# boyuanf/tensorflow_train_distributed

Measured on AMD Instinct MI355X. Metric: images/sec (whole node) ResNet-50 bf16 MirroredStrategy at 1/2/4/8 MI355X, higher is better.
Workload: dtype bf16; 1 GPU; model=ResNet-50 v1.5, global_batch=1024, per_gpu_batch=1024, image_size=224, parallelism=dp1, optimizer=momentum-SGD 0.9, wd 5e-5, fp32 master, precision=bf16, hipgraph=True

## Files before the change

tensorflow_train_distributed_amd/csrc/kernels/conv_dgrad.hip:

```cpp
#include "gemm_conv.h"

TTDK_EXPORT int ttdk_conv_dgrad(const bf16_t* dy, const bf16_t* wt, const TtdkConv* g, int bm, int bn,
                                const TtdkEpilogue* epi, hipStream_t st) {
  if (g->K % 8) return hipErrorInvalidValue;
  EpiParams pe = to_epi(epi);
  if (pe.by && (pe.stat == nullptr || pe.mode != 0 || g->C % 8 || pe.ldo % 8 || pe.residual || pe.act))
    return hipErrorInvalidValue;
  if ((pe.by2 || pe.stat2) && !(pe.by && pe.by2 && pe.stat2)) return hipErrorInvalidValue;
  const int N = g->C, K = g->R * g->S * g->K;
  DenseParams pb{wt, K, N, K};
  if (g->R == 1 && g->S == 1 && g->ph == 0 && g->pw == 0) {
    const int M = g->N * g->P * g->Q;
    DenseParams pa{dy, g->K, M, K};
    if (g->sh != 1 || g->sw != 1) {
      if (g->sh != g->sw || pe.bH) return hipErrorInvalidValue;
      pe.remap = 1;
      pe.rP = g->P;
      pe.rQ = g->Q;
      pe.rOH = g->H;
      pe.rOW = g->W;
      pe.rs = g->sh;
    }
    const int bbn = big_bn(M, N, K);
    if (((bm == 0 && pe.stat == nullptr) || bm == 256) && bbn && (bm != 256 || bn == bbn))
      return bbn == 256 ? big::dense<256>(dy, g->K, true, wt, K, true, pe, M, N, K, 1, st)
                        : big::dense<128>(dy, g->K, true, wt, K, true, pe, M, N, K, 1, st);
    if (bm == 256 && pe.stat) return hipErrorInvalidValue;
    if (bm == 0 || bn == 0 || bm == 256) pick_tile(M, N, &bm, &bn);
    return dispatch<KDense, KDense>(&pa, &pb, pe, M, N, K, 1, bm, bn, st);
  }
  const int M = g->N * g->H * g->W;
  const int bbn = big_bn(M, N, K);
  static const bool strided_big = [] {
    const char* e = getenv("TTD_BIG_STRIDED_DGRAD");
    return e != nullptr && e[0] == '1';
  }();
  const bool unit = g->sh == 1 && g->sw == 1;
  if (((bm == 0 && pe.stat == nullptr) || bm == 256) && bbn && (bm != 256 || bn == bbn) && g->K % 64 == 0 &&
      !pe.remap && (unit || strided_big)) {
    const big::ConvP pa = conv_params(dy, g->P, g->Q, g->K, g->H, g->W, g, M);
    const big::DenseP pb2{wt, K, N};
    if (unit) {
      if (bbn == 256)
        return big::launch<256, big::OpConvK<128, 2, true, true>, big::OpDenseK<128, 2>>(pa, pb2, pe, M, N, K, 1, st);
      return big::launch<128, big::OpConvK<128, 2, true, true>, big::OpDenseK<64, 2>>(pa, pb2, pe, M, N, K, 1, st);
    }
    if (bbn == 256)
      return big::launch<256, big::OpConvK<128, 2, true>, big::OpDenseK<128, 2>>(pa, pb2, pe, M, N, K, 1, st);
    return big::launch<128, big::OpConvK<128, 2, true>, big::OpDenseK<64, 2>>(pa, pb2, pe, M, N, K, 1, st);
  }
  if (bm == 256 && pe.stat) return hipErrorInvalidValue;
  if (bm == 0 || bn == 0 || bm == 256) pick_tile(M, N, &bm, &bn);
  GatherParams pa{dy, g->P, g->Q, g->K, g->H, g->W, g->R, g->S, g->sh, g->sw, g->ph, g->pw, g->dh, g->dw, M, K};
  return dispatch<KConvDgrad, KDense>(&pa, &pb, pe, M, N, K, 1, bm, bn, st);
}

TTDK_EXPORT int ttdk_conv_dgrad_bnpro(const bf16_t* g_in, const bf16_t* wt, const TtdkConv* g, const bf16_t* y,
                                      const float* coef, bf16_t* dz, const TtdkEpilogue* epi, hipStream_t st) {
  if (!plan::conv_dgrad_bnpro_takes(*g)) return hipErrorNotSupported;
  EpiParams pe = to_epi(epi);
  if (pe.by && (pe.stat == nullptr || pe.mode != 0 || g->C % 8 || pe.ldo % 8 || pe.residual || pe.act))
    return hipErrorInvalidValue;
  if ((pe.by2 || pe.stat2) && !(pe.by && pe.by2 && pe.stat2)) return hipErrorInvalidValue;
  const int N = g->C, K = g->K;
  const int M = g->N * g->P * g->Q;
  const int bbn = big_bn(M, N, K);
  if (pe.mode != 0 || pe.remap) return hipErrorNotSupported;
  pe.py = y;
  pe.pcoef = coef;
  pe.pdz = dz;
  pe.pld = K;
  const big::DenseP pa{g_in, K, M}, pb{wt, K, N};
  if (bbn == 256)
    return big::launch<256, big::OpDenseKBN<128, 2>, big::OpDenseK<128, 2>, 0, 0>(pa, pb, pe, M, N, K, 1, st);
  return big::launch<128, big::OpDenseKBN<128, 2>, big::OpDenseK<64, 2>, 0, 0>(pa, pb, pe, M, N, K, 1, st);
}

__global__ __launch_bounds__(256) void subpixel_weights_kernel(const bf16_t* __restrict__ wt, bf16_t* __restrict__ ws,
                                                               int C, int R, int S, int Kc, int s, int r0, int Tr,
                                                               int s0, int Ts) {
  const int k8n = Kc >> 3;
  const long long total = static_cast<long long>(C) * Tr * Ts * k8n;
  for (long long idx = blockIdx.x * 256LL + threadIdx.x; idx < total; idx += static_cast<long long>(gridDim.x) * 256) {
    const int k8 = static_cast<int>(idx % k8n);
    long long rest = idx / k8n;
    const int ts = static_cast<int>(rest % Ts);
    rest /= Ts;
    const int tr = static_cast<int>(rest % Tr);
    const long long c = rest / Tr;
    const bf16_t* src = wt + c * (static_cast<long long>(R) * S * Kc) +
                        (static_cast<long long>(r0 + tr * s) * S + (s0 + ts * s)) * Kc + k8 * 8;
    reinterpret_cast<uint4*>(ws)[idx] = *reinterpret_cast<const uint4*>(src);
  }
}

TTDK_EXPORT int ttdk_conv_dgrad_subpixel(const bf16_t* dy, const bf16_t* wt, const TtdkConv* g, bf16_t* ws,
                                         int ws_ready, const TtdkEpilogue* epi, hipStream_t st) {
  const int s = g->sh;
  if (g->sw != s || s < 2 || g->dh != 1 || g->dw != 1 || g->R < s || g->S < s || g->K % 8 || g->C % 8)
    return hipErrorInvalidValue;
  EpiParams pe = to_epi(epi);
  if (pe.remap || pe.residual || pe.aux || pe.mode == 1 || pe.by2 || pe.stat2 || pe.bH) return hipErrorInvalidValue;
  if ((pe.stat != nullptr) != (pe.by != nullptr) || (pe.by && (pe.mode != 0 || g->C % 8 || pe.ldo % 8)))
    return hipErrorInvalidValue;
  const int N = g->C, Kc = g->K;
  const size_t esz = pe.mode == 0 ? sizeof(bf16_t) : sizeof(float);
// ... 47 lines not shown
```

tensorflow_train_distributed_amd/csrc/kernels/gemm_conv.h:

```cpp
#pragma once
#include "common.h"
#include "gemm_plan.h"

#include <algorithm>
#include <cstdlib>
#include <type_traits>

namespace ttdk_rt {
int& pers_flag();
int& reserved_cus();
int& fold_flag();
}

namespace ttdk {
namespace {

using plan::big_bn;
using plan::big_bn_wgrad;
using plan::pick_tile;

constexpr int BK = 64;
constexpr int NTHR = 256;

__device__ __forceinline__ int kmaj_off(int row, int chunk) { return row * 128 + ((chunk ^ ((row >> 1) & 7)) << 4); }
// ... 1819 lines not shown
        if (E.stat2) r8[j] += __shfl_xor(r8[j], o, 64);
      }
    }
    float* red = reinterpret_cast<float*>(smem + BM * PITCH);
    if (lane < CPR) {
#pragma unroll
      for (int j = 0; j < 8; ++j) {
        red[(wave * 3 + 0) * BN + c * 8 + j] = s8[j];
        red[(wave * 3 + 1) * BN + c * 8 + j] = q8[j];
        red[(wave * 3 + 2) * BN + c * 8 + j] = r8[j];
      }
    }
    __syncthreads();
    for (int t2 = tid; t2 < BN; t2 += T) {
      if (n0 + t2 < N) {
        float ss = 0.f, qq = 0.f, rr = 0.f;
#pragma unroll
        for (int k = 0; k < NW; ++k) {
          ss += red[(k * 3 + 0) * BN + t2];
          qq += red[(k * 3 + 1) * BN + t2];
          rr += red[(k * 3 + 2) * BN + t2];
        }
        E.stat[(static_cast<long long>(tile_m) * 2 + 0) * N + n0 + t2] = ss;
        E.stat[(static_cast<long long>(tile_m) * 2 + 1) * N + n0 + t2] = qq;
        if (E.stat2) {
          E.stat2[(static_cast<long long>(tile_m) * 2 + 0) * N + n0 + t2] = ss;
          E.stat2[(static_cast<long long>(tile_m) * 2 + 1) * N + n0 + t2] = rr;
        }
      }
    }
  }
}


constexpr int kEkBias = 1, kEkDGelu = 2, kEkBeta = 4, kEkAux = 8, kEkGelu = 16;

template <int EK, bool CHECK, int BNH, int WC>
__device__ __forceinline__ void pers_epi(const f32x4_t (&acc)[2][2][4][2], const EpiParams& E, int m0, int n0, int M,
                                         int N, float alpha, int lane, int wm, int wn) {
  const int g = lane >> 4, i16 = lane & 15;
  const bool odd = g & 1;
  bf16_t* const out = static_cast<bf16_t*>(E.out);
  constexpr bool LD = (EK & (kEkDGelu | kEkBeta)) != 0;
  uint2 rvb[2][2][2], ovb[2][2][2];
  auto load_blk = [&](int it, uint2 (&rv)[2][2], uint2 (&ov)[2][2]) {
    const int ha = it >> 2, a = it & 3;
    const int m = m0 + ha * 128 + wm * 64 + a * 16 + i16;
    if (CHECK && m >= M) return;
#pragma unroll
    for (int hb = 0; hb < 2; ++hb) {
      const int nb = n0 + hb * BNH + wn * WC + 4 * g;
#pragma unroll
      for (int b = 0; b < 2; ++b) {
        if constexpr ((EK & kEkDGelu) != 0)
          if (!CHECK || nb + 16 * b < N)
            rv[hb][b] = *reinterpret_cast<const uint2*>(E.residual + static_cast<long long>(m) * E.ldr + nb + 16 * b);
        if constexpr ((EK & kEkBeta) != 0)
          if (!CHECK || nb + 16 * b < N)
            ov[hb][b] = *reinterpret_cast<const uint2*>(out + static_cast<long long>(m) * E.ldo + nb + 16 * b);
      }
    }
  };
  if constexpr (LD) load_blk(0, rvb[0], ovb[0]);
#pragma unroll
  for (int it = 0; it < 8; ++it) {
    const int ha = it >> 2, a = it & 3;
// ... 208 lines not shown
    if (atomicAdd(tq + 8, 1) == static_cast<int>(gridDim.x) - 1) {
#pragma unroll
      for (int i = 0; i < 9; ++i) tq[i] = 0;
    }
  }
}

constexpr int kMaxCtr = 1 << 16;
inline int* tile_counters(hipStream_t st, int tiles) {
  if (tiles > kMaxCtr - 16) return nullptr;
  struct Buf {
    hipStream_t st;
    int* p;
  };
  static Buf bufs[16] = {};
  for (auto& b : bufs)
    if (b.p && b.st == st) return b.p;
  for (auto& b : bufs) {
    if (!b.p) {
      if (hipMalloc(&b.p, kMaxCtr * sizeof(int)) != hipSuccess) return b.p = nullptr, nullptr;
      if (hipMemsetAsync(b.p, 0, kMaxCtr * sizeof(int), st) != hipSuccess) return nullptr;
      b.st = st;
      return b.p;
    }
  }
  return nullptr;
}

inline bool inkernel_fold() { return ::ttdk_rt::fold_flag() != 0; }

inline int device_cus_total() {
  static int cus = [] {
    int dev = 0, n = 0;
    hipGetDevice(&dev);
    if (hipDeviceGetAttribute(&n, hipDeviceAttributeMultiprocessorCount, dev) != hipSuccess || n <= 0) n = 256;
    return n;
  }();
  return cus;
}

inline int device_cus() {
  const int total = device_cus_total();
  const int r = ::ttdk_rt::reserved_cus();
  return (r > 0 && total - r >= total / 2) ? total - r : total;
}

template <int BN, class OA, class OB, int F8 = 0, int PP = 0>
hipError_t launch(const typename OA::Params& pa, const typename OB::Params& pb, const EpiParams& pe, int M, int N,
                  int K, int splits, hipStream_t st) {
  const int tm = ceil_div(M, BM), tn = ceil_div(N, BN);
  const int ktiles = K / (F8 ? 128 : 64);
  const int cus = device_cus();
  const int tiles = tm * tn;
  splits = plan::clamp_splits(ktiles, splits);
  const int per = ceil_div(ktiles, splits);
  if constexpr (F8 == 0 && PP == 1 && OA::THREADS == THR && BN == 256) {
    int ek = -1;
    if (pe.act == kActNone && !pe.residual) ek = 0;
    else if (pe.act == kActGelu && !pe.residual) ek = kEkGelu;
    else if (pe.act == kActDGelu && pe.residual) ek = kEkDGelu;
    if (ek >= 0) {
      if (pe.bias) ek |= kEkBias;
      if (pe.beta) ek |= kEkBeta;
      if (pe.aux) ek |= kEkAux;
    }
    if (::ttdk_rt::pers_flag() && splits == 1 && pe.mode == 0 && !pe.remap && !pe.stat && !pe.by && !pe.bH && tiles > cus &&
        N % 8 == 0 && pe.ldo % 8 == 0 && (!pe.residual || pe.ldr % 4 == 0) && (!pe.bias || al16(pe.bias)) &&
        al16(pe.out) && (!pe.aux || al16(pe.aux)) && (!pe.residual || (reinterpret_cast<uintptr_t>(pe.residual) & 7) == 0)) {
      const int ovl = ::ttdk_rt::pers_flag() == 1;
      static const int fullwait = getenv_int("TTD_PERS_STORE_WAIT", 0);
      static const int queue = getenv_int("TTD_PERS_QUEUE", 1);
      int* tq = nullptr;
      if (queue && cus % 8 == 0) {
        int* c = tile_counters(st, 0);
        if (c) tq = c + kMaxCtr - 16;
      }
#define TTDK_PERS(EKV)                                                                                                \
  case EKV:                                                                                                           \
    hipLaunchKernelGGL((gemm256p_kernel<BN, OA, OB, EKV>), dim3(cus), dim3(THR), 0, st, pa, pb, pe, M, N, K, tm, tn, ovl, \
                       fullwait, tq);                                                                                 \
    return hipGetLastError();
      switch (ek) {
        TTDK_PERS(0)
        TTDK_PERS(kEkBias)
        TTDK_PERS(kEkBias | kEkAux | kEkGelu)
        TTDK_PERS(kEkDGelu)
        TTDK_PERS(kEkBeta)
        default: break;
      }
#undef TTDK_PERS
    }
  }
  hipLaunchKernelGGL((gemm256_kernel<BN, OA, OB, F8, PP>), dim3(tm * tn, splits), dim3(OA::THREADS), 0, st, pa, pb, pe, M, N,
                     K, tm, tn, per, 0);
  return hipGetLastError();
}

template <int BN, int PP>
hipError_t dense_pp(const bf16_t* A, long long lda, bool ak, const bf16_t* B, long long ldb, bool bk,
                    const EpiParams& pe, int M, int N, int K, int splits, hipStream_t st) {
  DenseP pa{A, lda, M}, pb{B, ldb, N};
  constexpr int BH = BN / 2;
  if (ak && bk) return launch<BN, OpDenseK<128, 2>, OpDenseK<BH, 2>, 0, PP>(pa, pb, pe, M, N, K, splits, st);
  if (ak) return launch<BN, OpDenseKU<128, 2>, OpDenseMN<BH>, 0, PP>(pa, pb, pe, M, N, K, splits, st);
  if (bk) return launch<BN, OpDenseMN<128>, OpDenseKU<BH, 2>, 0, PP>(pa, pb, pe, M, N, K, splits, st);
  return launch<BN, OpDenseMN<128>, OpDenseMN<BH>, 0, PP>(pa, pb, pe, M, N, K, splits, st);
}

inline hipError_t dense_rowsum(const bf16_t* A, long long lda, const bf16_t* B, long long ldb, const EpiParams& pe,
                               int M, int N, int K, int splits, hipStream_t st) {
  DenseP pa{A, lda, M}, pb{B, ldb, N};
  const int tm = ceil_div(M, BM), tn = ceil_div(N, 256);
  const int ktiles = K / 64;
  splits = plan::clamp_splits(ktiles, splits);
  const int per = ceil_div(ktiles, splits);
  hipLaunchKernelGGL((gemm256_kernel<256, OpDenseMN<128>, OpDenseMN<128>, 0, 1, 1>), dim3(tm * tn, splits), dim3(THR), 0,
                     st, pa, pb, pe, M, N, K, tm, tn, per, 0);
  return hipGetLastError();
}

template <int BN>
hipError_t dense(const bf16_t* A, long long lda, bool ak, const bf16_t* B, long long ldb, bool bk,
                 const EpiParams& pe, int M, int N, int K, int splits, hipStream_t st) {
  if constexpr (BN == 256) {
    static const int pp_on = getenv_int("TTD_BIG_PP", 1);
    const int kts = K / 64 / (splits > 1 ? splits : 1);
    if (kts >= 16 && pp_on)
// ... 131 lines not shown
```

tensorflow_train_distributed_amd/csrc/kernels/gemm_plan.h:

```cpp
#pragma once

struct TtdkConv {
  int N, H, W, C;
  int K, R, S;
  int P, Q;
  int sh, sw, ph, pw, dh, dw;
};

namespace ttdk {
namespace plan {

inline int cdiv(long long a, long long b) { return static_cast<int>((a + b - 1) / b); }

inline bool is_pointwise(const TtdkConv& g) {
  return g.R == 1 && g.S == 1 && g.sh == 1 && g.sw == 1 && g.ph == 0 && g.pw == 0;
}
inline bool unit_no_dilation(const TtdkConv& g) { return g.sh == 1 && g.sw == 1 && g.dh == 1 && g.dw == 1; }
inline long long out_pixels(const TtdkConv& g) { return static_cast<long long>(g.N) * g.P * g.Q; }
inline long long in_pixels(const TtdkConv& g) { return static_cast<long long>(g.N) * g.H * g.W; }

inline int big_bn(int M, int N, int K) {
  if (M < 256 || N < 128 || K % 64 || N % 8 || static_cast<long long>(M) * N < (1LL << 20)) return 0;
  return N >= 256 ? 256 : 128;
}
// ... 90 lines not shown
           yb + shift >= (1LL << 31) || (N + 256) * K * 2 >= (1LL << 32));
}
inline bool conv_fwd4k8_takes(const TtdkConv& g) {
  const long long M = out_pixels(g), N = g.K, K = static_cast<long long>(g.R) * g.S * g.C;
  const long long xb = in_pixels(g) * g.C;
  const long long shift = (static_cast<long long>(g.ph) * g.W + g.pw) * g.C;
  if (g.C % 128 || N % 8 || N < 8 || M < 1 || g.dh != 1 || g.dw != 1 || g.R * g.S > 32 ||
      xb + shift >= (1LL << 31) || (N + 256) * K >= (1LL << 32))
    return false;
  return !(is_pointwise(g) && M * g.C >= (1LL << 32));
}
inline bool conv_dgrad4k8_takes(const TtdkConv& g) {
  const long long M = in_pixels(g), N = g.C, K = static_cast<long long>(g.R) * g.S * g.K;
  const long long yb = out_pixels(g) * g.K;
  const int pho = g.R - 1 - g.ph, pwo = g.S - 1 - g.pw;
  const long long shift = (static_cast<long long>(pho) * g.Q + pwo) * g.K;
  return !(!unit_no_dilation(g) || g.K % 128 || N % 8 || N < 8 || g.R * g.S > 32 || pho < 0 || pwo < 0 || M < 1 ||
           yb + shift >= (1LL << 31) || (N + 256) * K >= (1LL << 32));
}
inline bool conv_wgrad_fp8_takes(const TtdkConv& g) {
  const long long M = g.K, N = static_cast<long long>(g.R) * g.S * g.C, K = out_pixels(g);
  return !(g.C % 16 || g.K % 16 || K % 128 || N < 256 || M < 16 || in_pixels(g) * g.C >= (1LL << 32));
}
inline bool conv_wgrad_bn_takes(const TtdkConv& g) {
  return !(g.C % 8 || g.K % 8 || is_pointwise(g) ||
           big_bn_wgrad(g.K, g.R * g.S * g.C, static_cast<int>(out_pixels(g))));
}
inline bool conv_dgrad_bnpro_takes(const TtdkConv& g) {
  return is_pointwise(g) && g.K % 64 == 0 && big_bn(static_cast<int>(out_pixels(g)), g.C, g.K) != 0;
}
inline bool conv_fwd_bnpro_takes(const TtdkConv& g) {
  return is_pointwise(g) && g.C % 64 == 0 && big_bn(static_cast<int>(out_pixels(g)), g.K, g.C) != 0;
}
inline bool gemm4t_takes(long long M, long long N, long long K) {
  return !(K % 64 || K < 128 || M < 8 || N < 8 || M % 8 || N % 8 || K * M * 2 >= (1LL << 31) ||
           K * N * 2 >= (1LL << 31));
}
inline bool conv_wgrad4t_takes(const TtdkConv& g) {
  const long long K = out_pixels(g);
  if (g.C % 8 || g.K % 8 || K % 64 || K < 128 || g.dh != 1 || g.dw != 1 || in_pixels(g) * g.C * 2 >= (1LL << 31) ||
      K * g.K * 2 >= (1LL << 31) || g.P * g.Q < 2 || g.Q < 2)
    return false;
  return gemm4t_takes(g.K, static_cast<long long>(g.R) * g.S * g.C, K);
}
inline bool conv_wgrad4t8_takes(const TtdkConv& g) {
  const long long M = g.K, N = static_cast<long long>(g.R) * g.S * g.C, K = out_pixels(g);
  return !(g.C % 16 || g.K % 16 || M < 16 || N < 16 || K % 128 || K < 128 || g.dh != 1 || g.dw != 1 ||
           in_pixels(g) * g.C >= (1LL << 31) || K * g.K >= (1LL << 31) ||
           (!is_pointwise(g) && (g.P * g.Q < 2 || g.Q < 2)));
}

}
}
```

tensorflow_train_distributed_amd/csrc/runtime/gemm_plan.cc:

```cpp
#include "../kernels/gemm_plan.h"

#include "common.h"

namespace plan = ttdk::plan;

TTD_EXPORT int ttd_plan_conv_size() { return static_cast<int>(sizeof(TtdkConv)); }

TTD_EXPORT int ttd_plan_big_bn(int M, int N, int K) { return plan::big_bn(M, N, K); }
TTD_EXPORT int ttd_plan_big_bn_wgrad(int M, int N, int K) { return plan::big_bn_wgrad(M, N, K); }
TTD_EXPORT void ttd_plan_pick_tile(int M, int N, int* bm, int* bn) { plan::pick_tile(M, N, bm, bn); }
TTD_EXPORT int ttd_plan_g4t_bm(int M, int rowsum, int bm128_enabled) {
  return plan::g4t_bm(M, rowsum != 0, bm128_enabled != 0);
}

TTD_EXPORT int ttd_plan_clamp_splits(int ktiles, int splits) { return plan::clamp_splits(ktiles, splits); }
TTD_EXPORT int ttd_plan_clamp_splits_4t(int ktiles, int splits) { return plan::clamp_splits_4t(ktiles, splits); }

TTD_EXPORT int ttd_plan_phase_pair(const TtdkConv* g, int idx, int* out) {
  plan::Phase r, c;
  const bool any = plan::phase_pair(*g, idx, &r, &c);
  const int v[8] = {r.r0, r.T, r.off, r.n, c.r0, c.T, c.off, c.n};
  std::memcpy(out, v, sizeof(v));
  return any;
}

TTD_EXPORT void ttd_plan_dgrad_stat(const TtdkConv* g, int stat_4w_k, int* bm, int* bn, int* rows) {
  plan::dgrad_stat_plan(*g, stat_4w_k, bm, bn, rows);
}
TTD_EXPORT long long ttd_plan_subpixel_stat_rows(const TtdkConv* g) { return plan::subpixel_stat_rows(*g); }

#define TTD_PLAN_TAKES(NAME) \
  TTD_EXPORT int ttd_plan_##NAME##_takes(const TtdkConv* g) { return plan::NAME##_takes(*g); }
TTD_PLAN_TAKES(conv_fwd4w)
TTD_PLAN_TAKES(conv_dgrad4w)
TTD_PLAN_TAKES(conv_fwd4k8)
TTD_PLAN_TAKES(conv_dgrad4k8)
TTD_PLAN_TAKES(conv_wgrad_fp8)
TTD_PLAN_TAKES(conv_wgrad_bn)
TTD_PLAN_TAKES(conv_dgrad_bnpro)
TTD_PLAN_TAKES(conv_fwd_bnpro)
TTD_PLAN_TAKES(conv_wgrad4t)
TTD_PLAN_TAKES(conv_wgrad4t8)
#undef TTD_PLAN_TAKES
TTD_EXPORT int ttd_plan_gemm4t_takes(long long M, long long N, long long K) { return plan::gemm4t_takes(M, N, K); }
```

tensorflow_train_distributed_amd/models/resnet.py:

```python
from __future__ import annotations

import math
import os
from dataclasses import dataclass
from typing import List, Optional

import numpy as np
import torch
import torch.nn.functional as F

from ..train.flat import FlatParams, ParamSpec
from ..utils import graphs

STAGES_50 = ((64, 3, 1), (128, 4, 2), (256, 6, 2), (512, 3, 2))


def _he_init(fan_in):
    std = math.sqrt(2.0 / fan_in) / 0.87962566103423978

    def init(t, gen):
        t.normal_(0.0, std, generator=gen)
        t.clamp_(-2 * std, 2 * std)
    init.dev = (1, 0.0, std)
    return init
# ... 175 lines not shown
            for key in ("c3", "c2", "cd", "c1"):
                if blk[key] is not None:
                    specs += self._conv_specs(blk[key])
        specs += self._conv_specs(self.stem)
        stem_k = specs[-5]
        base_init = stem_k.init
        cin = self.in_channels

        def stem_init(t, gen, base_init=base_init, cin=cin):
            base_init(t, gen)
            t[..., cin:] = 0.0
        stem_k.init = stem_init
        return specs

    def conv_list(self) -> List[ConvSpec]:
        out = [self.stem]
        for blk in self.blocks:
            out += [blk[k] for k in ("c1", "c2", "c3", "cd") if blk[k] is not None]
        return out

    def _pw_fwd_ok(self, c: ConvSpec, fused_input: bool) -> bool:
        from ..ops import gemm as G
        if not (self.fuse_pw and self.device.type == "cuda" and c.k == 1 and c.stride == 1 and c.pad == 0):
            return False
        if not G.pw_ok(1 << 20, c.cout, c.cin_store):
            return False
        return c.cin_store <= 128 or (fused_input and c.cin_store == 256)

    def _pw_part(self, name):
        return self.fuse_pw and self.pw_parts.get(name, True)

    PW_DGRAD_SHAPES = {(256, 64), (64, 256)}

    BNPRO_MAX_K = 1024
    BNPRO_MAX_N = 512
    FWDPRO_MAX_K = 512

    def _fwd_pro_ok(self, c: ConvSpec, x_shape) -> bool:
        from ..ops import gemm as G
        return (self.fwd_pro and self.device.type == "cuda" and c.k == 1 and c.stride == 1 and c.pad == 0
                and c.cin_store <= self.FWDPRO_MAX_K and c.cout <= self.BNPRO_MAX_N and not self._fp8_conv(c)
                and G.conv_fwd_bnpro_ok(tuple(x_shape), (c.cout, 1, 1, c.cin_store)))

    def _pw_dgrad_ok(self, c: ConvSpec) -> bool:
        from ..ops import gemm as G
        return (self.fuse_pw and self.device.type == "cuda" and c.k == 1 and c.stride == 1 and c.pad == 0
                and (c.cout, c.cin_store) in self.PW_DGRAD_SHAPES and G.pw_ok(1 << 20, c.cin_store, c.cout))

    def _stem_packed_ok(self, shape) -> bool:
        from ..ops import gemm as G
        c = self.stem
        w = (c.cout, c.k, c.k, c.cin_store)
        from ..ops import kernels as K
        return (self.device.type == "cuda" and self.stem_fwd_kernel and self.stem_kernel and self.fuse_bn_bwd
                and shape[-1] == self.in_channels and K.stem_pool_fusable((shape[0], 112, 112, c.cout))
                and G.stem_fwd_ok(shape, w, (c.stride, c.stride), (c.pad, c.pad), self.in_channels)
                and G.stem_wgrad_ok(shape, w, (c.stride, c.stride), (c.pad, c.pad), self.in_channels))

    def _c3_ok(self, c: ConvSpec, H: int, W: int) -> bool:
        from ..ops import gemm as G
        return (self.fuse_c3 and self.device.type == "cuda" and c.k == 3 and c.stride == 1 and c.pad == 1
                and G.conv3_rows(H, W, c.cin_store, c.cout) > 0)

    def _convbn_fwd(self, c: ConvSpec, x, relu, residual=None, x8=None, want8=False, pool=False, defer=False,
                    residual_bn=None, pro=None, pro_big=False, store_out=True):
        from ..ops import gemm as G
        from ..ops import kernels as K
        P = self.params
        N, H, W, C = x.shape
        Pp = (H + 2 * c.pad - c.k) // c.stride + 1
        Q = (W + 2 * c.pad - c.k) // c.stride + 1
        M = N * Pp * Q
        bm = 128 if M > 64 else 64
        bn = 128 if c.cout > 64 else 64
# ... 607 lines not shown
```

tensorflow_train_distributed_amd/ops/_lib.py:

```python
from __future__ import annotations

import ctypes
from ctypes import c_float, c_int, c_longlong, c_uint64, c_void_p

import torch

from .. import _native

P = c_void_p
I = c_int
L = c_longlong
F = c_float
U64 = c_uint64


class Epilogue(ctypes.Structure):

    _fields_ = [
        ("mode", c_int), ("out", c_void_p), ("ldo", c_longlong), ("slab_stride", c_longlong),
        ("bias", c_void_p), ("residual", c_void_p), ("ldr", c_longlong), ("act", c_int),
        ("beta", c_int), ("remap", c_int), ("rP", c_int), ("rQ", c_int), ("rOH", c_int),
        ("rOW", c_int), ("rs", c_int), ("stat", c_void_p), ("alpha", c_float), ("aux", c_void_p),
        ("ascale0", c_void_p), ("ascale1", c_void_p), ("by", c_void_p), ("bmask", c_void_p),
        ("by2", c_void_p), ("stat2", c_void_p), ("bH", c_int), ("bW", c_int),
    ]


class ConvGeom(ctypes.Structure):

    _fields_ = [(n, c_int) for n in ("N", "H", "W", "C", "K", "R", "S", "P", "Q", "sh", "sw", "ph", "pw", "dh", "dw")]


class DwConvGeom(ctypes.Structure):

    _fields_ = [(n, c_int) for n in ("N", "H", "W", "C", "M", "R", "S", "P", "Q", "sh", "sw", "ph", "pw", "dh", "dw")]


E = ctypes.POINTER(Epilogue)
G = ctypes.POINTER(ConvGeom)
DG = ctypes.POINTER(DwConvGeom)

_SIGS = {
    "ttdk_gemm_bf16": [P, L, I, P, L, I, I, I, I, I, I, I, E, P],
    "ttdk_gemm_bf16_splitk": [P, L, I, P, L, I, I, I, I, I, P, P, I, F, I, I, P],
    "ttdk_gemm_wgrad_bias": [P, L, P, L, I, I, I, I, P, P, I, F, P, P],
    "ttdk_gemm_wgrad_bias_ws": [I, I, I, I],
    "ttdk_gemm4t_wgrad": [P, L, P, L, I, I, I, I, P, P, I, F, P, P],
    "ttdk_gemm4t_ws": [I, I, I, I],
    "ttdk_conv_fwd": [P, P, G, I, I, E, P],
    "ttdk_conv_fwd4w": [P, P, G, E, P],
    "ttdk_conv_dgrad4w": [P, P, G, E, P],
    "ttdk_conv_dgrad": [P, P, G, I, I, E, P],
    "ttdk_conv_dgrad_bnpro": [P, P, G, P, P, P, E, P],
    "ttdk_set_inkernel_fold": [I],
    "ttdk_conv_fwd_bnpro": [P, P, G, P, P, I, P, P, E, P],
    "ttdk_conv_dgrad_subpixel": [P, P, G, P, I, E, P],
    "ttdk_conv_wgrad": [P, P, G, P, P, I, I, I, I, P],
    "ttdk_conv_wgrad4t": [P, P, G, P, P, I, I, P],
    "ttdk_conv_wgrad4t_ws": [G, I],
    "ttdk_conv_wgrad_bn": [P, P, P, P, G, P, P, I, I, I, I, P],
    "ttdk_conv_wgrad_fp8": [P, P, G, P, P, I, I, P, P, P],
    "ttdk_conv_wgrad4t8": [P, P, G, P, P, I, I, P, P, P],
    "ttdk_conv_fwd4k8": [P, P, G, P, P, P, P, P],
    "ttdk_conv_dgrad4k8": [P, P, G, P, P, P, P, I, P, P, P],
    "ttdk_conv_wgrad4t8_ws": [G, I],
    "ttdk_splitk_reduce": [P, I, L, P, I, P],
    "ttdk_set_big_pers": [I],
    "ttdk_gemm_f32": [P, L, I, P, L, I, P, L, P, I, I, I, I, P],
    "ttdk_stem_fwd_blocks": [I],
    "ttdk_stem_fwd": [P, P, P, P, I, I, I, I, P],
    "ttdk_stem_wgrad_blocks": [I, I, I],
    "ttdk_stem_wgrad": [P, P, P, P, P, P, I, I, I, I, I, I, I, P],
    "ttdk_conv3_rows": [I, I, I, I, I],
    "ttdk_conv3_halo": [P, P, P, P, P, P, P, I, I, P, I, I, I, I, I, E, P],
    "ttdk_pw_rows": [I, I, I],
    "ttdk_pw_conv": [P, P, P, P, P, P, P, P, P, I, I, P, L, I, I, I, E, P],
    "ttdk_pw_wgrad_slabs": [I, I, I, I, I],
    "ttdk_pw_conv_wgrad": [P, P, P, P, P, P, L, I, I, I, E, P, P, I, I, P],
    "ttdk_bn_num_partials": [L, I],
    "ttdk_bn_stats_partial": [P, L, I, P, I, P],
    "ttdk_bn_bwd_partial": [P, P, P, P, L, I, P, I, P, P],
    "ttdk_bn_reduce_partials": [P, I, I, P, P],
    "ttdk_bn_fwd_finalize": [P, F, I, P, P, F, F, P, P, P, P, P, P, P],
    "ttdk_bn_finalize_slices": [I],
    "ttdk_bn_reduce_finalize": [P, I, I, P, I, F, P, P, F, F, P, P, P, P, P, P, P, P, P, I, P],
    "ttdk_bn_bwd_finalize": [P, F, I, P, P, P, P, P, P, I, P],
# ... 101 lines not shown
```

tensorflow_train_distributed_amd/ops/_plan.py:

```python
from __future__ import annotations

import ctypes
from collections import namedtuple
from ctypes import c_int, c_longlong

from .. import _native
from ._lib import DG, ConvGeom, DwConvGeom, G

_PI = ctypes.POINTER(c_int)
_TAKES = ("conv_fwd4w", "conv_dgrad4w", "conv_fwd4k8", "conv_dgrad4k8", "conv_wgrad_fp8", "conv_wgrad_bn",
          "conv_dgrad_bnpro", "conv_fwd_bnpro", "conv_wgrad4t", "conv_wgrad4t8")
_SIGS = {
    "conv_size": (c_int, []),
    "big_bn": (c_int, [c_int] * 3),
    "big_bn_wgrad": (c_int, [c_int] * 3),
    "pick_tile": (None, [c_int, c_int, _PI, _PI]),
    "g4t_bm": (c_int, [c_int] * 3),
    "clamp_splits": (c_int, [c_int] * 2),
    "clamp_splits_4t": (c_int, [c_int] * 2),
    "phase_pair": (c_int, [G, c_int, _PI]),
    "dgrad_stat": (None, [G, c_int, _PI, _PI, _PI]),
    "subpixel_stat_rows": (c_longlong, [G]),
    "gemm4t_takes": (c_int, [c_longlong] * 3),
}
_SIGS.update({n + "_takes": (c_int, [G]) for n in _TAKES})
_PL = ctypes.POINTER(c_longlong)
_DW_SIGS = {
    "geom_size": (c_int, []),
    "valid": (c_int, [DG]),
    "fast_takes": (c_int, [DG, c_int]),
    "strip": (c_int, []),
    "max_slabs": (c_int, []),
    "wgrad_parts": (c_int, [DG]),
    "slab_rows": (None, [DG, c_int, _PL, _PL]),
    "part_stride": (c_longlong, [DG]),
    "wgrad_ws_floats": (c_longlong, [DG]),
}

_fns = {}


def _fn(name):
    if not _fns:
        lib = _native.rt()
        for n, (res, args) in _SIGS.items():
            f = getattr(lib, "ttd_plan_" + n)
            f.restype, f.argtypes = res, args
            _fns[n] = f
        if _fns["conv_size"]() != ctypes.sizeof(ConvGeom):
            raise RuntimeError("ops._lib.ConvGeom (%d bytes) does not match TtdkConv (%d bytes)"
                               % (ctypes.sizeof(ConvGeom), _fns["conv_size"]()))
    return _fns[name]


def pick_tile(M, N):
    bm, bn = c_int(), c_int()
    _fn("pick_tile")(M, N, bm, bn)
    return bm.value, bn.value


Phase = namedtuple("Phase", "r0 T off n")


def subpixel_phases(g):
    out = []
    v = (c_int * 8)()
    for i in range(g.sh * g.sh):
        if _fn("phase_pair")(ctypes.byref(g), i, v):
            out.append((Phase(*v[:4]), Phase(*v[4:])))
    return out


def dgrad_stat(g, stat_4w_k):
    bm, bn, rows = c_int(), c_int(), c_int()
    _fn("dgrad_stat")(ctypes.byref(g), stat_4w_k, bm, bn, rows)
    return bm.value, bn.value, rows.value


def takes(launcher, g) -> bool:
    return bool(_fn(launcher + "_takes")(ctypes.byref(g)))


def _direct(name):
    return lambda *args: _fn(name)(*args)


big_bn, big_bn_wgrad, g4t_bm, clamp_splits, clamp_splits_4t, gemm4t_takes = map(
    _direct, ("big_bn", "big_bn_wgrad", "g4t_bm", "clamp_splits", "clamp_splits_4t", "gemm4t_takes"))


def subpixel_stat_rows(g):
    return _fn("subpixel_stat_rows")(ctypes.byref(g))


_dw_fns = {}


def _dw(name):
    if not _dw_fns:
        lib = _native.rt()
        for n, (res, args) in _DW_SIGS.items():
            f = getattr(lib, "ttd_dwplan_" + n)
            f.restype, f.argtypes = res, args
            _dw_fns[n] = f
        if _dw_fns["geom_size"]() != ctypes.sizeof(DwConvGeom):
            raise RuntimeError("ops._lib.DwConvGeom (%d bytes) does not match TtdkDwConv (%d bytes)"
                               % (ctypes.sizeof(DwConvGeom), _dw_fns["geom_size"]()))
    return _dw_fns[name]

# ... 40 lines not shown
```

tensorflow_train_distributed_amd/ops/gemm.py:

```python
from __future__ import annotations

import ctypes

import torch

from . import _lib, _plan

ACT_NONE, ACT_RELU, ACT_GELU, ACT_TANH, ACT_DGELU = 0, 1, 2, 3, 4

import os as _os
_LOG = [] if _os.environ.get("TTD_GEMM_LOG") else None


def gemm_log(reset=False):
    out = list(_LOG or [])
    if reset and _LOG is not None:
        _LOG.clear()
    return out


def _log(kind, M, N, K, splits=1):
    if _LOG is not None:
        _LOG.append((kind, int(M), int(N), int(K), int(splits)))
    _lib.label((kind, int(M), int(N), int(K)))
# ... 516 lines not shown
    ws = torch.empty_like(wt) if ws is None else ws
    _lib.call("ttdk_conv_dgrad_subpixel", dy.data_ptr(), wt.data_ptr(), ctypes.byref(g), ws.data_ptr(), int(ready),
              ctypes.byref(e), _lib.stream())


def _subpixel_ok(g, R, S, stride, padding):
    return (_SUBPIXEL and not (R == 1 and S == 1 and tuple(padding) == (0, 0)) and g.sh == g.sw and g.sh > 1
            and R >= g.sh and S >= g.sw)


def dgrad_stat_rows(x_shape, wt_shape, stride=(1, 1), padding=(0, 0)):
    C, R, S, K = wt_shape
    N, H, W, _ = x_shape
    if C % 8:
        return None
    if tuple(stride) != (1, 1):
        g = conv_geom(tuple(x_shape), (K, R, S, C), stride, padding)
        if not _subpixel_ok(g, R, S, stride, padding):
            return None
        return _plan.subpixel_stat_rows(g)
    return dgrad_stat_tile(x_shape, wt_shape)[2]


DGRAD_STAT_4W_K = int(_os.environ.get("TTD_DGRAD_STAT_4W_K", "0"))


def dgrad_stat_tile(x_shape, wt_shape, stride=(1, 1), padding=(0, 0)):
    C, R, S, K = wt_shape
    if tuple(stride) != (1, 1):
        return None
    return _plan.dgrad_stat(conv_geom(tuple(x_shape), (K, R, S, C), stride, padding), DGRAD_STAT_4W_K)


def _bnpro_call(dy, wt, g, bn_pro, e):
    y, coef, dz = bn_pro
    C, R, S, K = wt.shape
    if not _plan.takes("conv_dgrad_bnpro", g):
        raise ValueError("conv_dgrad: the BN-backward operand prologue needs a 1x1 unit-stride dgrad on the 256-row "
                         "kernel")
    _check(y, torch.bfloat16, "bn_pro y")
    _check(dz, torch.bfloat16, "bn_pro dz")
    if tuple(y.shape) != tuple(dy.shape) or tuple(dz.shape) != tuple(dy.shape) or coef.dtype != torch.float32 \
            or coef.numel() != 3 * K or not coef.is_contiguous():
        raise ValueError("conv_dgrad: bn_pro operands must match dy ([..., K]) and coef [3, K] fp32")
    _log("dgrad_bnpro_1x1", g.N * g.H * g.W, C, K)
    _lib.call("ttdk_conv_dgrad_bnpro", dy.data_ptr(), wt.data_ptr(), ctypes.byref(g), y.data_ptr(), coef.data_ptr(),
              dz.data_ptr(), ctypes.byref(e), _lib.stream())


def dgrad_bnpro_ok(x_shape, wt_shape, stride=(1, 1), padding=(0, 0)):
    C, R, S, K = wt_shape
    return _plan.takes("conv_dgrad_bnpro", conv_geom(tuple(x_shape), (K, R, S, C), stride, padding))


def conv_dgrad(dy, wt, x_shape, stride=(1, 1), padding=(0, 0), *, out=None, beta=0, residual=None,
               tile=(0, 0), bn_stat=None, bn_stat2=None, sampled_only=False, beta_s2=None, bn_pro=None, ws=None):
    _check(dy, torch.bfloat16, "dy")
    _check(wt, torch.bfloat16, "wt")
    if beta_s2 is not None and beta and tuple(stride) != (1, 1):
        raise ValueError("conv_dgrad: beta_s2 needs a unit-stride dgrad")
    C, R, S, K = wt.shape
    g = conv_geom(x_shape, (K, R, S, C), stride, padding)
    strided_pw = R == 1 and S == 1 and padding == (0, 0) and tuple(stride) != (1, 1)
    if out is None:
        alloc = torch.zeros if (strided_pw and not beta and not sampled_only) else torch.empty
        out = alloc(tuple(x_shape), dtype=torch.bfloat16, device=dy.device)
    if bn_stat is not None:
        y, mask = bn_stat
        T = dgrad_stat_rows(tuple(x_shape), tuple(wt.shape), stride, padding)
        if T is None or residual is not None or tuple(y.shape) != tuple(x_shape):
            raise ValueError("conv_dgrad: BN-statistics epilogue not available for this conv")
        _check(y, torch.bfloat16, "bn_stat y")
        partial = torch.empty((T, 2, C), dtype=torch.float32, device=dy.device)
        partial2 = None
        if bn_stat2 is not None:
            _check(bn_stat2, torch.bfloat16, "bn_stat2")
            if tuple(bn_stat2.shape) != tuple(x_shape) or tuple(stride) != (1, 1):
                raise ValueError("conv_dgrad: second BN statistics need a unit-stride dgrad of the same shape")
            partial2 = torch.empty((T, 2, C), dtype=torch.float32, device=dy.device)
        e = _epi(out, ldo=C, beta=beta, stat=partial, by=y, bmask=mask, by2=bn_stat2, stat2=partial2,
                 beta_s2=beta_s2 if beta else None)
        if tuple(stride) != (1, 1):
            _subpixel_call(dy, wt, g, ws, e)
        elif bn_pro is not None:
            _bnpro_call(dy, wt, g, bn_pro, e)
        elif (not beta and partial2 is None and residual is None
              and conv_dgrad4w_pays(tuple(x_shape), tuple(wt.shape), stride, padding)):
            T = 2 * -(-(g.N * g.H * g.W) // 256)
            partial = torch.empty((T, 2, C), dtype=torch.float32, device=dy.device)
            e = _epi(out, ldo=C, stat=partial, by=y, bmask=mask)
            _log("dgrad4w_%dx%d_s1" % (R, S), g.N * g.H * g.W, C, R * S * K)
            _lib.call("ttdk_conv_dgrad4w", dy.data_ptr(), wt.data_ptr(), ctypes.byref(g), ctypes.byref(e),
                      _lib.stream())
        else:
            bm, bn, _ = dgrad_stat_tile(tuple(x_shape), tuple(wt.shape))
            _log("dgrad_%dx%d_s%d" % (R, S, stride[0]), g.N * g.H * g.W, C, R * S * K)
            _lib.call("ttdk_conv_dgrad", dy.data_ptr(), wt.data_ptr(), ctypes.byref(g), bm, bn, ctypes.byref(e),
                      _lib.stream())
        return (out, partial, T) if partial2 is None else (out, partial, T, partial2)
    e = _epi(out, ldo=C, beta=beta, residual=residual, beta_s2=beta_s2 if beta else None)
    if bn_pro is not None:
        _bnpro_call(dy, wt, g, bn_pro, e)
# ... 340 lines not shown
```

Measured before the change: 16030 images/sec.

## Add two-workgroup-per-CU BN-prologue dgrad kernel and widen bnpro eligibility

Adds a new 128-row, 256-thread GEMM kernel for the 1x1 dgrad with fused BN-backward operand prologue. Its LDS footprint is sized so two workgroups fit per CU. The planner selects it by default when C >= 256, and the ResNet BNPRO size limits are raised so larger pointwise convs also take the fused prologue path. The aim is more overlap between the prologue transform and the MFMA work, plus fewer separate BN-backward passes. The trade-offs are smaller tiles, more redundant y and coef loads across N tiles, and a single-buffered pipeline.

```diff
diff --git a/tensorflow_train_distributed_amd/csrc/kernels/conv_dgrad.hip b/tensorflow_train_distributed_amd/csrc/kernels/conv_dgrad.hip
--- a/tensorflow_train_distributed_amd/csrc/kernels/conv_dgrad.hip
+++ b/tensorflow_train_distributed_amd/csrc/kernels/conv_dgrad.hip
@@ -56,22 +56,25 @@
 }
 
 TTDK_EXPORT int ttdk_conv_dgrad_bnpro(const bf16_t* g_in, const bf16_t* wt, const TtdkConv* g, const bf16_t* y,
-                                      const float* coef, bf16_t* dz, const TtdkEpilogue* epi, hipStream_t st) {
-  if (!plan::conv_dgrad_bnpro_takes(*g)) return hipErrorNotSupported;
+                                      const float* coef, bf16_t* dz, int form, const TtdkEpilogue* epi,
+                                      hipStream_t st) {
+  const plan::DgradBnpro pl = plan::dgrad_bnpro_plan(*g, form);
+  if (!pl.form) return hipErrorNotSupported;
   EpiParams pe = to_epi(epi);
   if (pe.by && (pe.stat == nullptr || pe.mode != 0 || g->C % 8 || pe.ldo % 8 || pe.residual || pe.act))
     return hipErrorInvalidValue;
   if ((pe.by2 || pe.stat2) && !(pe.by && pe.by2 && pe.stat2)) return hipErrorInvalidValue;
   const int N = g->C, K = g->K;
   const int M = g->N * g->P * g->Q;
-  const int bbn = big_bn(M, N, K);
   if (pe.mode != 0 || pe.remap) return hipErrorNotSupported;
   pe.py = y;
   pe.pcoef = coef;
   pe.pdz = dz;
   pe.pld = K;
   const big::DenseP pa{g_in, K, M}, pb{wt, K, N};
-  if (bbn == 256)
+  if (pl.form == 2)
+    return pl.bn == 256 ? big::launch_kbn2wg<256>(pa, pb, pe, M, N, K, st) : big::launch_kbn2wg<128>(pa, pb, pe, M, N, K, st);
+  if (pl.bn == 256)
     return big::launch<256, big::OpDenseKBN<128, 2>, big::OpDenseK<128, 2>, 0, 0>(pa, pb, pe, M, N, K, 1, st);
   return big::launch<128, big::OpDenseKBN<128, 2>, big::OpDenseK<64, 2>, 0, 0>(pa, pb, pe, M, N, K, 1, st);
 }
diff --git a/tensorflow_train_distributed_amd/csrc/kernels/gemm_conv.h b/tensorflow_train_distributed_amd/csrc/kernels/gemm_conv.h
--- a/tensorflow_train_distributed_amd/csrc/kernels/gemm_conv.h
+++ b/tensorflow_train_distributed_amd/csrc/kernels/gemm_conv.h
@@ -1875,6 +1875,230 @@
   }
 }
 
+constexpr int BM2 = 128, THR2 = 256;
+
+template <int BN>
+struct Geo2 {
+  static constexpr int BNH = BN / 2;
+  static constexpr int AH = BM2 * 128;
+  static constexpr int BH = BNH * 128;
+  static constexpr int STAGE = AH + 2 * BH;
+  static constexpr int COEF = STAGE;
+  static constexpr int PITCH = BN * 2 + 16;
+  static constexpr int EPI = BM2 * PITCH + 4 * 3 * BN * 4;
+  static constexpr int SMEM = (STAGE + 1024 > EPI) ? STAGE + 1024 : EPI;
+};
+
+template <int ROWS>
+struct Rows2 {
+  static constexpr int G = ROWS * 8 / THR2;
+  long long base;
+  int off[G];
+  __device__ __forceinline__ void init(const DenseP& P, int row0, int tid) {
+    const int chunk = (tid & 7) ^ ((tid >> 4) & 7);
+    const int rb = min(row0, P.rows - 1);
+    base = static_cast<long long>(rb) * P.ld * 2 + chunk * 16;
+#pragma unroll
+    for (int i = 0; i < G; ++i)
+      off[i] = (min(row0 + ((i * THR2 + tid) >> 3), P.rows - 1) - rb) * static_cast<int>(P.ld) * 2;
+  }
+  __device__ __forceinline__ void issue(const void* p, char* lds, int kt, int wave) const {
+    const char* s = static_cast<const char*>(p) + base + static_cast<long long>(kt) * 128;
+#pragma unroll
+    for (int i = 0; i < G; ++i) glds(s + off[i], lds + (i * THR2 + wave * 64) * 16);
+  }
+};
+
+template <int BN>
+__global__ __launch_bounds__(THR2, 2) void kbn2wg_kernel(DenseP pa, DenseP pb, EpiParams E, int M, int N, int K,
+                                                         int tiles_m, int tiles_n) {
+  using Gm = Geo2<BN>;
+  using OA = Rows2<BM2>;
+  using OB = Rows2<BN>;
+  constexpr int T = THR2, NW = T / 64, WN = 2;
+  constexpr int BNH = Gm::BNH, WC = BNH / WN, NB = WC / 16, GA = OA::G;
+  static_assert(2 * Gm::SMEM <= 160 * 1024, "two workgroups per CU");
+  __shared__ __attribute__((aligned(16))) char smem[Gm::SMEM];
+  const int t = xcd_remap(blockIdx.x, tiles_m * tiles_n);
+  const int tile_n = t % tiles_n, tile_m = t / tiles_n;
+  const int m0 = tile_m * BM2, n0 = tile_n * BN;
+  const int tid = threadIdx.x, lane = tid & 63, wave = tid >> 6;
+  const int wm = wave / WN, wn = wave % WN;
+
+  OA la;
+  OB lb;
+  la.init(pa, m0, tid);
+  lb.init(pb, n0, tid);
+
+  f32x4_t acc[2][4][NB];
+#pragma unroll
+  for (int hb = 0; hb < 2; ++hb)
+#pragma unroll
+    for (int a = 0; a < 4; ++a)
+#pragma unroll
+      for (int b = 0; b < NB; ++b) acc[hb][a][b] = f32x4_t{0.f, 0.f, 0.f, 0.f};
+
+  constexpr int A0 = 0, B0 = Gm::AH, B1 = Gm::AH + Gm::BH;
+  const int ktiles = K / 64;
+  uint4 yv[GA];
+  const int pchunk = (tid & 7) ^ ((tid >> 4) & 7);
+  auto prow = [&](int i) { return m0 + ((i * T + tid) >> 3); };
+  auto load_tile = [&](int kt) {
+    const char* ys = reinterpret_cast<const char*>(E.py) + la.base + static_cast<long long>(kt) * 128;
+#pragma unroll
+    for (int i = 0; i < GA; ++i) yv[i] = *reinterpret_cast<const uint4*>(ys + la.off[i]);
+    const float* src = lane < 48 ? E.pcoef + static_cast<long long>(lane >> 4) * K + kt * 64 + (lane & 15) * 4
+                                 : reinterpret_cast<const float*>(g_zero);
+    if (wave == 0) glds(src, smem + Gm::COEF);
+    la.issue(pa.p, smem + A0, kt, wave);
+    lb.issue(pb.p, smem + B0, kt, wave);
+  };
+  auto transform = [&](int kt) {
+    const float* cf = reinterpret_cast<const float*>(smem + Gm::COEF) + pchunk * 8;
+    float c0[8], c1[8], c2[8];
+#pragma unroll
+    for (int j = 0; j < 8; j += 4) {
+      *reinterpret_cast<f32x4_t*>(c0 + j) = *reinterpret_cast<const f32x4_t*>(cf + j);
+      *reinterpret_cast<f32x4_t*>(c1 + j) = *reinterpret_cast<const f32x4_t*>(cf + 64 + j);
+      *reinterpret_cast<f32x4_t*>(c2 + j) = *reinterpret_cast<const f32x4_t*>(cf + 128 + j);
+    }
+    const bool store = tile_n == 0;
+    char* zs = reinterpret_cast<char*>(E.pdz) + la.base + static_cast<long long>(kt) * 128;
+#pragma unroll
+    for (int i = 0; i < GA; ++i) {
+      uint4* q = reinterpret_cast<uint4*>(smem + A0 + (i * T + tid) * 16);
+      float gv[8], yf[8];
+      unpack8(*q, gv);
+      unpack8(yv[i], yf);
+#pragma unroll
+      for (int j = 0; j < 8; ++j) gv[j] = c0[j] * gv[j] + c1[j] * yf[j] + c2[j];
+      const uint4 o = pack8(gv);
+      *q = o;
+      if (store && prow(i) < M) *reinterpret_cast<uint4*>(zs + la.off[i]) = o;
+    }
+  };
+
+  bf16x8_t fa[4], fb[2][NB];
+  auto read_k = [&](int ks) {
+#pragma unroll
+    for (int a = 0; a < 4; ++a) fa[a] = frag_k(smem + A0, wm * 64 + a * 16, ks, lane);
+#pragma unroll
+    for (int hb = 0; hb < 2; ++hb)
+#pragma unroll
+      for (int b = 0; b < NB; ++b) fb[hb][b] = frag_k(smem + (hb ? B1 : B0), wn * WC + b * 16, ks, lane);
+  };
+  auto mma = [&]() {
+    __builtin_amdgcn_s_setprio(1);
+#pragma unroll
+    for (int hb = 0; hb < 2; ++hb)
+#pragma unroll
+      for (int a = 0; a < 4; ++a)
+#pragma unroll
+        for (int b = 0; b < NB; ++b)
+          acc[hb][a][b] = __builtin_amdgcn_mfma_f32_16x16x32_bf16(fb[hb][b], fa[a], acc[hb][a][b], 0, 0, 0);
+    __builtin_amdgcn_s_setprio(0);
+  };
+  load_tile(0);
+  for (int kt = 0; kt < ktiles; ++kt) {
+    wait_vm<0>();
+    barrier();
+    transform(kt);
+    barrier();
+    read_k(0);
+    mma();
+    __builtin_amdgcn_sched_barrier(0);
+    read_k(1);
+    if (kt + 1 < ktiles) {
+      asm volatile("s_waitcnt lgkmcnt(0)" ::: "memory");
+      barrier();
+      load_tile(kt + 1);
+    }
+    mma();
+  }
+  wait_vm<0>();
+  __syncthreads();
+
+  const int g = lane >> 4, i16 = lane & 15;
+  const float alpha_e = epi_alpha(E);
+  constexpr int PITCH = Gm::PITCH;
+  constexpr int CPR = BN / 8;
+  constexpr int RPP = T / CPR;
+  const int c = tid % CPR, r0 = tid / CPR;
+  const int n = n0 + c * 8;
+  auto stage = [&](auto HB) {
+    constexpr int hb = decltype(HB)::value;
+#pragma unroll
+    for (int a = 0; a < 4; ++a)
+#pragma unroll
+      for (int b = 0; b < NB; ++b) {
+        const int r = wm * 64 + a * 16 + i16, cc = hb * BNH + wn * WC + b * 16 + 4 * g;
+        const f32x4_t v = acc[hb][a][b] * alpha_e;
+        *reinterpret_cast<uint2*>(smem + r * PITCH + cc * 2) =
+            make_uint2(pack_bf16x2(v[0], v[1]), pack_bf16x2(v[2], v[3]));
+      }
+  };
+  float s8[8], q8[8], r8[8];
+#pragma unroll
+  for (int j = 0; j < 8; ++j) s8[j] = q8[j] = r8[j] = 0.f;
+  const bool feed = E.feed_pf && E.by && !E.residual && !E.bias && E.act == kActNone && !E.remap &&
+                    !E.aux && E.stat;
+  if (feed) {
+    feed_epilogue<BM2 / RPP, RPP, PITCH, false>(E, smem, stage, c, r0, m0, M, n, N, s8, q8, r8);
+  } else {
+    stage(std::integral_constant<int, 0>{});
+    stage(std::integral_constant<int, 1>{});
+    __syncthreads();
+    const bool nfull = n + 8 <= N;
+    const bool vst = nfull && (E.ldo & 7) == 0;
+    const bool vres = nfull && (E.ldr & 7) == 0;
+    float bias8[8];
+#pragma unroll
+    for (int j = 0; j < 8; ++j) bias8[j] = (E.bias && n + j < N) ? E.bias[n + j] : 0.f;
+    if (E.beta || E.residual || E.by)
+      epi_rows<BM2, RPP, PITCH, true, 4>(E, smem, c, r0, n, m0, M, N, vst, vres, bias8, s8, q8, r8);
+    else
+      epi_rows<BM2, RPP, PITCH, false>(E, smem, c, r0, n, m0, M, N, vst, vres, bias8, s8, q8, r8);
+  }
+  if (E.stat) {
+#pragma unroll
+    for (int j = 0; j < 8; ++j) {
+#pragma unroll
+      for (int o = CPR; o < 64; o <<= 1) {
+        s8[j] += __shfl_xor(s8[j], o, 64);
+        q8[j] += __shfl_xor(q8[j], o, 64);
+        if (E.stat2) r8[j] += __shfl_xor(r8[j], o, 64);
+      }
+    }
+    float* red = reinterpret_cast<float*>(smem + BM2 * PITCH);
+    if (lane < CPR) {
+#pragma unroll
+      for (int j = 0; j < 8; ++j) {
+        red[(wave * 3 + 0) * BN + c * 8 + j] = s8[j];
+        red[(wave * 3 + 1) * BN + c * 8 + j] = q8[j];
+        red[(wave * 3 + 2) * BN + c * 8 + j] = r8[j];
+      }
+    }
+    __syncthreads();
+    for (int t2 = tid; t2 < BN; t2 += T) {
+      if (n0 + t2 < N) {
+        float ss = 0.f, qq = 0.f, rr = 0.f;
+#pragma unroll
+        for (int k = 0; k < NW; ++k) {
+          ss += red[(k * 3 + 0) * BN + t2];
+          qq += red[(k * 3 + 1) * BN + t2];
+          rr += red[(k * 3 + 2) * BN + t2];
+        }
+        E.stat[(static_cast<long long>(tile_m) * 2 + 0) * N + n0 + t2] = ss;
+        E.stat[(static_cast<long long>(tile_m) * 2 + 1) * N + n0 + t2] = qq;
+        if (E.stat2) {
+          E.stat2[(static_cast<long long>(tile_m) * 2 + 0) * N + n0 + t2] = ss;
+          E.stat2[(static_cast<long long>(tile_m) * 2 + 1) * N + n0 + t2] = rr;
+        }
+      }
+    }
+  }
+}
+
 
 constexpr int kEkBias = 1, kEkDGelu = 2, kEkBeta = 4, kEkAux = 8, kEkGelu = 16;
 
@@ -2149,8 +2373,9 @@
 inline int device_cus_total() {
   static int cus = [] {
     int dev = 0, n = 0;
-    hipGetDevice(&dev);
-    if (hipDeviceGetAttribute(&n, hipDeviceAttributeMultiprocessorCount, dev) != hipSuccess || n <= 0) n = 256;
+    if (hipGetDevice(&dev) != hipSuccess ||
+        hipDeviceGetAttribute(&n, hipDeviceAttributeMultiprocessorCount, dev) != hipSuccess || n <= 0)
+      n = 256;
     return n;
   }();
   return cus;
@@ -2210,6 +2435,14 @@
   }
   hipLaunchKernelGGL((gemm256_kernel<BN, OA, OB, F8, PP>), dim3(tm * tn, splits), dim3(OA::THREADS), 0, st, pa, pb, pe, M, N,
                      K, tm, tn, per, 0);
+  return hipGetLastError();
+}
+
+template <int BN>
+hipError_t launch_kbn2wg(const DenseP& pa, const DenseP& pb, const EpiParams& pe, int M, int N, int K,
+                         hipStream_t st) {
+  const int tm = ceil_div(M, BM2), tn = ceil_div(N, BN);
+  hipLaunchKernelGGL((kbn2wg_kernel<BN>), dim3(tm * tn), dim3(THR2), 0, st, pa, pb, pe, M, N, K, tm, tn);
   return hipGetLastError();
 }
 
diff --git a/tensorflow_train_distributed_amd/csrc/kernels/gemm_plan.h b/tensorflow_train_distributed_amd/csrc/kernels/gemm_plan.h
--- a/tensorflow_train_distributed_amd/csrc/kernels/gemm_plan.h
+++ b/tensorflow_train_distributed_amd/csrc/kernels/gemm_plan.h
@@ -146,6 +146,31 @@
 inline bool conv_fwd_bnpro_takes(const TtdkConv& g) {
   return is_pointwise(g) && g.C % 64 == 0 && big_bn(static_cast<int>(out_pixels(g)), g.K, g.C) != 0;
 }
+inline int dgrad_bnpro_form(int M, int N, int K) {
+  (void)M;
+  (void)K;
+  return N >= 256 ? 2 : 1;
+}
+struct DgradBnpro {
+  int form, bm, bn, rows;
+};
+inline DgradBnpro dgrad_bnpro_plan(const TtdkConv& g, int force) {
+  DgradBnpro p{0, 0, 0, 0};
+  const long long M = out_pixels(g);
+  if (!is_pointwise(g) || g.K < 64 || g.K % 64 || g.K >= (1 << 22) || g.C < 8 || g.C % 8 || M < 1 ||
+      M >= (1LL << 31) - 256)
+    return p;
+  if (force == 1 || force == 2) {
+    p.form = force;
+  } else {
+    if (!conv_dgrad_bnpro_takes(g)) return p;
+    p.form = dgrad_bnpro_form(static_cast<int>(M), g.C, g.K);
+  }
+  p.bm = p.form == 2 ? 128 : 256;
+  p.bn = g.C >= 256 ? 256 : 128;
+  p.rows = cdiv(M, p.bm);
+  return p;
+}
 inline bool gemm4t_takes(long long M, long long N, long long K) {
   return !(K % 64 || K < 128 || M < 8 || N < 8 || M % 8 || N % 8 || K * M * 2 >= (1LL << 31) ||
            K * N * 2 >= (1LL << 31));
diff --git a/tensorflow_train_distributed_amd/csrc/runtime/gemm_plan.cc b/tensorflow_train_distributed_amd/csrc/runtime/gemm_plan.cc
--- a/tensorflow_train_distributed_amd/csrc/runtime/gemm_plan.cc
+++ b/tensorflow_train_distributed_amd/csrc/runtime/gemm_plan.cc
@@ -27,6 +27,11 @@
 TTD_EXPORT void ttd_plan_dgrad_stat(const TtdkConv* g, int stat_4w_k, int* bm, int* bn, int* rows) {
   plan::dgrad_stat_plan(*g, stat_4w_k, bm, bn, rows);
 }
+TTD_EXPORT void ttd_plan_dgrad_bnpro(const TtdkConv* g, int force, int* out) {
+  const plan::DgradBnpro p = plan::dgrad_bnpro_plan(*g, force);
+  const int v[4] = {p.form, p.bm, p.bn, p.rows};
+  std::memcpy(out, v, sizeof(v));
+}
 TTD_EXPORT long long ttd_plan_subpixel_stat_rows(const TtdkConv* g) { return plan::subpixel_stat_rows(*g); }
 
 #define TTD_PLAN_TAKES(NAME) \
diff --git a/tensorflow_train_distributed_amd/models/resnet.py b/tensorflow_train_distributed_amd/models/resnet.py
--- a/tensorflow_train_distributed_amd/models/resnet.py
+++ b/tensorflow_train_distributed_amd/models/resnet.py
@@ -231,14 +231,15 @@
 
     PW_DGRAD_SHAPES = {(256, 64), (64, 256)}
 
-    BNPRO_MAX_K = 1024
-    BNPRO_MAX_N = 512
+    BNPRO_MAX_K = 2048
+    BNPRO_MAX_N = 2048
     FWDPRO_MAX_K = 512
+    FWDPRO_MAX_N = 512
 
     def _fwd_pro_ok(self, c: ConvSpec, x_shape) -> bool:
         from ..ops import gemm as G
         return (self.fwd_pro and self.device.type == "cuda" and c.k == 1 and c.stride == 1 and c.pad == 0
-                and c.cin_store <= self.FWDPRO_MAX_K and c.cout <= self.BNPRO_MAX_N and not self._fp8_conv(c)
+                and c.cin_store <= self.FWDPRO_MAX_K and c.cout <= self.FWDPRO_MAX_N and not self._fp8_conv(c)
                 and G.conv_fwd_bnpro_ok(tuple(x_shape), (c.cout, 1, 1, c.cin_store)))
 
     def _pw_dgrad_ok(self, c: ConvSpec) -> bool:
diff --git a/tensorflow_train_distributed_amd/ops/_lib.py b/tensorflow_train_distributed_amd/ops/_lib.py
--- a/tensorflow_train_distributed_amd/ops/_lib.py
+++ b/tensorflow_train_distributed_amd/ops/_lib.py
@@ -51,7 +51,7 @@
     "ttdk_conv_fwd4w": [P, P, G, E, P],
     "ttdk_conv_dgrad4w": [P, P, G, E, P],
     "ttdk_conv_dgrad": [P, P, G, I, I, E, P],
-    "ttdk_conv_dgrad_bnpro": [P, P, G, P, P, P, E, P],
+    "ttdk_conv_dgrad_bnpro": [P, P, G, P, P, P, I, E, P],
     "ttdk_set_inkernel_fold": [I],
     "ttdk_conv_fwd_bnpro": [P, P, G, P, P, I, P, P, E, P],
     "ttdk_conv_dgrad_subpixel": [P, P, G, P, I, E, P],
diff --git a/tensorflow_train_distributed_amd/ops/_plan.py b/tensorflow_train_distributed_amd/ops/_plan.py
--- a/tensorflow_train_distributed_amd/ops/_plan.py
+++ b/tensorflow_train_distributed_amd/ops/_plan.py
@@ -20,6 +20,7 @@
     "clamp_splits_4t": (c_int, [c_int] * 2),
     "phase_pair": (c_int, [G, c_int, _PI]),
     "dgrad_stat": (None, [G, c_int, _PI, _PI, _PI]),
+    "dgrad_bnpro": (None, [G, c_int, _PI]),
     "subpixel_stat_rows": (c_longlong, [G]),
     "gemm4t_takes": (c_int, [c_longlong] * 3),
 }
@@ -75,6 +76,15 @@
     bm, bn, rows = c_int(), c_int(), c_int()
     _fn("dgrad_stat")(ctypes.byref(g), stat_4w_k, bm, bn, rows)
     return bm.value, bn.value, rows.value
+
+
+DgradBnpro = namedtuple("DgradBnpro", "form bm bn rows")
+
+
+def dgrad_bnpro(g, force=0):
+    v = (c_int * 4)()
+    _fn("dgrad_bnpro")(ctypes.byref(g), force, v)
+    return DgradBnpro(*v)
 
 
 def takes(launcher, g) -> bool:
diff --git a/tensorflow_train_distributed_amd/ops/gemm.py b/tensorflow_train_distributed_amd/ops/gemm.py
--- a/tensorflow_train_distributed_amd/ops/gemm.py
+++ b/tensorflow_train_distributed_amd/ops/gemm.py
@@ -572,10 +572,13 @@
     return _plan.dgrad_stat(conv_geom(tuple(x_shape), (K, R, S, C), stride, padding), DGRAD_STAT_4W_K)
 
 
+DGRAD_BNPRO_FORM = int(_os.environ.get("TTD_DGRAD_BNPRO_FORM", "0"))
+
+
 def _bnpro_call(dy, wt, g, bn_pro, e):
     y, coef, dz = bn_pro
     C, R, S, K = wt.shape
-    if not _plan.takes("conv_dgrad_bnpro", g):
+    if not _plan.dgrad_bnpro(g, DGRAD_BNPRO_FORM).form:
         raise ValueError("conv_dgrad: the BN-backward operand prologue needs a 1x1 unit-stride dgrad on the 256-row "
                          "kernel")
     _check(y, torch.bfloat16, "bn_pro y")
@@ -585,12 +588,12 @@
         raise ValueError("conv_dgrad: bn_pro operands must match dy ([..., K]) and coef [3, K] fp32")
     _log("dgrad_bnpro_1x1", g.N * g.H * g.W, C, K)
     _lib.call("ttdk_conv_dgrad_bnpro", dy.data_ptr(), wt.data_ptr(), ctypes.byref(g), y.data_ptr(), coef.data_ptr(),
-              dz.data_ptr(), ctypes.byref(e), _lib.stream())
+              dz.data_ptr(), DGRAD_BNPRO_FORM, ctypes.byref(e), _lib.stream())
 
 
 def dgrad_bnpro_ok(x_shape, wt_shape, stride=(1, 1), padding=(0, 0)):
     C, R, S, K = wt_shape
-    return _plan.takes("conv_dgrad_bnpro", conv_geom(tuple(x_shape), (K, R, S, C), stride, padding))
+    return _plan.dgrad_bnpro(conv_geom(tuple(x_shape), (K, R, S, C), stride, padding), DGRAD_BNPRO_FORM).form != 0
 
 
 def conv_dgrad(dy, wt, x_shape, stride=(1, 1), padding=(0, 0), *, out=None, beta=0, residual=None,
@@ -608,6 +611,8 @@
     if bn_stat is not None:
         y, mask = bn_stat
         T = dgrad_stat_rows(tuple(x_shape), tuple(wt.shape), stride, padding)
+        if bn_pro is not None:
+            T = _plan.dgrad_bnpro(g, DGRAD_BNPRO_FORM).rows or T
         if T is None or residual is not None or tuple(y.shape) != tuple(x_shape):
             raise ValueError("conv_dgrad: BN-statistics epilogue not available for this conv")
         _check(y, torch.bfloat16, "bn_stat y")
```

Measured after the change: 16100 images/sec (median of 4 runs). Within noise of the previous version (+0.5%).
